# danspeech/danspeech

Hardware: AMD Instinct MI355X
Metric: audio-seconds/sec (RTFx) recognize() on 10 s clips, batch=32 (higher is better)
Workload: dtype f32 (two-term fp16 split operands, 3 MFMA products, fp32 accumulate)

## Files before the change

### danspeech_amd/_native.py

```python
import ctypes as C
import os

import numpy as np

_HERE = os.path.dirname(os.path.abspath(__file__))
LIB_PATH = os.environ.get("DSMI_LIBRARY") or os.path.join(_HERE, "lib", "libdsmi.so")

RNN_TYPES = {"gru": 0, "lstm": 1, "rnn": 2}
WINDOWS = {"hamming": 0, "hann": 1, "blackman": 2, "bartlett": 3}
PCM_DTYPES = {np.dtype(np.int16): 0, np.dtype(np.float32): 1, np.dtype(np.float64): 2}
WAV_WIDTH_DTYPE = {1: 3, 2: 0, 3: 4, 4: 5}
PCM_STEREO = 16
_PCM_BYTES = (2, 4, 8, 1, 3, 4)
PAD_MODES = {"reflect": 0, "constant": 1}
RESAMPLE_METHODS = {"polyphase": 0, "ratecv": 1}
RESAMPLE_STREAM_MAX = 256
ENDPOINT_MAX = 256
STREAM_MANY_MAX = 256
BEAM_STREAM_MANY_MAX = 4096
ALIGN_MAX_TOKENS = 4096
SPOT_MAX_TOKENS = 128
SPOT_MAX_PHRASES = 4096
SPOT_MAX_HITS = 64
SCORE_MAX_TOKENS = 2048
# ... 108 lines not shown
    "dsmi_rnn_layer": (C.c_int, [_vp, C.c_int, _vp, _vp, C.c_int, C.c_int, _vp, _vp]),
    "dsmi_head": (C.c_int, [_vp, _vp, _vp, C.c_int, C.c_int, _vp, _vp]),
    "dsmi_greedy": (C.c_int, [_vp, _vp, _vp, C.c_int, C.c_int, _vp, _vp, _vp, _vp]),
    "dsmi_greedy_enqueue": (C.c_int, [_vp, _vp, _vp, C.c_int, C.c_int, _vp]),
    "dsmi_greedy_collect": (C.c_int, [_vp, _vp, _vp, _vp]),
    "dsmi_set_profiling": (C.c_int, [_vp, C.c_int]),
    "dsmi_stage_time_us": (C.c_double, [_vp, C.c_int]),
    "dsmi_kernel_stats": (C.c_int, [_vp, C.c_int, _i64p, _i64p, C.POINTER(C.c_double), C.POINTER(C.c_double), C.POINTER(C.c_double)]),
    "dsmi_reset_kernel_stats": (C.c_int, [_vp]),
    "dsmi_debug_persist_stamps": (C.c_int, [_vp, C.c_int, C.c_int, C.c_int, _vp, C.c_int64]),
    "dsmi_debug_step_stamps": (C.c_int, [_vp, C.c_int, C.c_int, C.c_int, C.c_int, _vp, C.c_int64]),
    "dsmi_debug_last_rnn_plan": (C.c_int, [_vp, C.c_char_p, C.c_int64]),
    "dsmi_debug_xproj": (C.c_int, [_vp, _vp, C.c_int64, _vp, _vp, _vp]),
    "dsmi_debug_conv_workgroups": (C.c_int, [_vp, _vp, C.c_int32]),
    "dsmi_debug_dense_stamps": (C.c_int, [_vp, C.c_int64]),
    "dsmi_last_forward_stats": (C.c_int, [_vp, _i64p, C.POINTER(C.c_double), C.POINTER(C.c_double)]),
    "dsmi_lm_open": (C.c_int, [C.c_char_p, C.POINTER(_vp)]),
    "dsmi_lm_close": (None, [_vp]),
    "dsmi_lm_last_error": (C.c_char_p, [_vp]),
    "dsmi_lm_info": (C.c_int, [_vp, C.POINTER(C.c_int), _i64p, C.POINTER(C.c_int)]),
    "dsmi_lm_word_index": (C.c_int, [_vp, C.c_char_p]),
    "dsmi_lm_lookup": (C.c_int, [_vp, _vp, C.c_int, C.POINTER(C.c_float), C.POINTER(C.c_float)]),
    "dsmi_lm_cond_log10": (C.c_double, [_vp, _vp, C.c_int]),
    "dsmi_beam_enqueue": (C.c_int, [_vp, _vp, _vp, C.c_int, C.c_int, C.c_int, C.c_int, C.c_double, _vp]),
    "dsmi_beam_collect": (C.c_int, [_vp, _vp, _vp, _vp, _vp]),
    "dsmi_decoder_beam_stats": (C.c_int, [_vp, _vp]),
    "dsmi_debug_beam_stamps": (C.c_int, [_vp, _vp, C.c_int64]),
    "dsmi_beam_stream_create": (C.c_int, [_vp, C.c_int, C.c_int, C.c_double, C.POINTER(_vp)]),
    "dsmi_beam_stream_destroy": (None, [_vp]),
    "dsmi_beam_stream_last_error": (C.c_char_p, [_vp]),
# ... 1043 lines not shown
```

### danspeech_amd/csrc/api.hip

```cpp
#include "common.h"
#include "model.h"
#include "gate.h"

#include <algorithm>
#include <cstring>

using namespace dsmi;

static int check_lens(dsmi_model* m, const int32_t* lens, int B, int T) {
    for (int i = 0; i < B; ++i) {
        if (lens[i] < 1 || lens[i] > T) return fail(m, DSMI_ERR_INVALID, "length outside 1..T");
        if (i && lens[i] > lens[i - 1]) return fail(m, DSMI_ERR_UNSORTED, "`lengths` array must be sorted in decreasing order");
    }
    return DSMI_OK;
}

static int check_batch(dsmi_model* m, const int32_t* lens, int B, int T) {
    if (!m->finalized) return fail(m, DSMI_ERR_NOT_READY, "dsmi_model_finalize has not been called");
    if (!lens || B < 1 || T < 1) return fail(m, DSMI_ERR_INVALID, "bad batch arguments");
    return check_lens(m, lens, B, T);
}

static int run_conv(dsmi_model* m, const float* feat, int B, int T, int To, int ys, hipStream_t s, const float** out) {
    const float* x = feat;
// ... 72 lines not shown
        const char *k = std::getenv("DSMI_RNN_KERNEL"), *t = exp_env("DSMI_RING_TILES"), *c = exp_env("DSMI_DEBUG_RING_SLOTS");
        return RingEnv{k && std::string(k) == "ring4", t ? std::atoi(t) : 4, c ? std::atoi(c) : 0};
    }();
    return env;
}

static RnnPlanInput rnn_plan_input(const dsmi_model* m, int B, bool split16) {
    RnnPlanInput in;
    in.geom = m->geom; in.geom16 = m->geom16; in.have16 = m->have16; in.split16 = split16;
    in.B = B; in.n_cus = m->n_cus; in.inflight = m->inflight; in.ring_windows = m->ring_windows; in.lane = m->lane;
    in.rnn_mode = m->rnn_mode; in.persist_gen = m->persist_gen; in.rnn_kernel = m->rnn_kernel; in.ring8 = m->ring8; in.ring4 = m->ring4;
    in.ring4_small_shapes = ring_env().small_shapes; in.ring4_most = ring_env().most; in.ring_slot_cap = ring_env().slot_cap;
    return in;
}

static bool run_rnn_plan(dsmi_model* m, const RnnPlan& plan, int l, int B, int To, int dst, double sumlen, hipStream_t s) {
    const double H = m->desc.rnn_hidden_size, GH = (double)m->geom.G * m->desc.rnn_hidden_size, Dd = m->geom.D;
    if (plan.launches[0].kernel == RNN_STEPS) {
        RnnStepLaunch st = rnn_step_launch(m, l, B, To, dst);
        for (int step = 0; step < To; ++step) {
            st.step = step;
            int act = 0;
            for (int i = 0; i < B; ++i) act += step < m->host_out_lens[i] ? 1 : 0;
            st.ev = timer_arm(m, KK_STEP, (step & 7) == 3, 2.0 * Dd * GH * H * act, 4.0 * Dd * (GH * H + (double)B * (GH + 2.0 * H)));
            launch_rnn_step(st, s);
        }
        m->last_plan_x16 = false; m->last_plan_n = 1; m->last_plan[0] = plan.launches[0];
        return true;
    }
    RnnPersist16Launch p16;
    RnnPersistLaunch p8;
    if (plan.x16) p16 = persist16_launch(m, l, B, To, dst);
    else p8 = persist_launch(m, l, B, To, dst);
    const size_t cnt_words = persist_cnt_words(m, B, To, true, false);
    (void)hipMemsetAsync(m->pcnt, 0, sizeof(unsigned) * persist_cnt_words(m, B, To, plan.x16, true), s);
    static const bool ring_xcd = [] { const char* e = exp_env("DSMI_DEBUG_RING_XCD"); return !(e && e[0] == '0'); }();
    GateTurn turn;
    bool ok = true;
    for (int i = 0; i < plan.launches.size() && ok; ++i) {
        const RnnLaunch& L = plan.launches[i];
        const EvPair ev = timer_arm(m, KK_PERSIST, true, L.part * 2.0 * Dd * GH * H * sumlen, L.part * 4.0 * Dd * (GH * H + (double)To * B * (GH + 2.0 * H)));
        if (!L.join) turn.wait(m->device, s, L, m->n_cus);
        p16.ev = ev;
        switch (L.kernel) {
            case RNN_PERSIST8: p8.ev = ev; p8.d0 = L.at; p8.ny = L.n; ok = launch_rnn_persist(p8, s); break;
            case RNN_PERSIST16: p16.pgroups = L.n; p16.waves = 8; ok = launch_rnn_persist16(p16, s); break;
            case RNN_PERSIST16_HALF: p16.pgroups = L.n; p16.waves = 4; ok = launch_rnn_persist16(p16, s); break;
            case RNN_DUO: p16.pair0 = L.at; p16.npairs = L.n; ok = launch_rnn_persist_duo(p16, s); break;
            default:
                p16.tile0 = L.at; p16.ntw = L.n; p16.nwin = L.nwin;
                p16.tickets = ring_xcd ? m->pcnt + cnt_words + L.ticket : nullptr;
                ok = L.kernel == RNN_RING8 ? launch_rnn_persist_ring(p16, s) : launch_rnn_persist_ring4(p16, s);
        }
        if (!ok || i + 1 == plan.launches.size() || !plan.launches[i + 1].join) turn.record();
    }
    if (ok) {
        m->last_plan_x16 = plan.x16; m->last_plan_n = plan.launches.size();
        for (int i = 0; i < std::min(m->last_plan_n, (int)dsmi_model::kLastPlanKept); ++i) m->last_plan[i] = plan.launches[i];
    }
    return ok;
}

static void run_rnn_layer(dsmi_model* m, int l, GemmLaunch gl, int B, int To, int dst, hipStream_t s) {
    double sumlen = 0;
    for (int i = 0; i < B; ++i) sumlen += m->host_out_lens[i];
    const double GH = (double)m->geom.G * m->desc.rnn_hidden_size, Dd = m->geom.D;
    RnnPlanInput in = rnn_plan_input(m, B, m->gemm_mode == 1 && gl.w_sp);
    RnnPlan plan = plan_rnn_layer(in);
    if (plan.x16) {
        gl.w_sp = m->rnn[l].wih16_sp; gl.bias = m->rnn[l].bih16; gl.N = m->geom16.Np; gl.ldc = m->geom16.Np;
    }
    gl.ev = timer_arm(m, gl.mode == GEMM_A_CONV ? KK_GEMM0 : KK_GEMM, true, 2.0 * Dd * GH * gl.K * sumlen,
                      4.0 * ((double)gl.M * gl.K * (gl.a2 ? 2 : 1) + (double)gl.N * gl.K + (double)gl.M * gl.N));
    DenseHold hold(m->device, m->inflight, DENSE_GEMM, s);
    m->last_xp_wgs = launch_gemm(gl, s);
    m->last_xp_rows = gl.M; m->last_xp_cols = gl.ldc;
    hold.leave();
    if (run_rnn_plan(m, plan, l, B, To, dst, sumlen, s)) return;
    if (plan.x16) {
        gl.w_sp = m->rnn[l].wih_sp; gl.bias = m->rnn[l].bih; gl.N = m->geom.Np; gl.ldc = m->geom.Np; gl.ev = EvPair{};
        m->last_xp_wgs = launch_gemm(gl, s);
        m->last_xp_cols = gl.ldc;
        in.have16 = false;
        plan = plan_rnn_layer(in);
        if (run_rnn_plan(m, plan, l, B, To, dst, sumlen, s)) return;
    }
    in.rnn_mode = 0;
    (void)run_rnn_plan(m, plan_rnn_layer(in), l, B, To, dst, sumlen, s);
}

static GemmLaunch xproj_gemm(dsmi_model* m, int l, int B, int To) {
    GemmLaunch gl{};
    const RnnW& r = m->rnn[l];
// ... 303 lines not shown
```

### danspeech_amd/csrc/common.h

```cpp
#pragma once
#include <hip/hip_runtime.h>
#include <hip/hip_ext.h>
#include <atomic>
#include <cstdint>
#include <cstdio>
#include <cstdlib>
#include <string>
#include <vector>
#include <map>

#include "../../include/dsmi.h"
#include "dense_tiles.h"
#include "conv_rows.h"
#include "rnn_plan.h"

namespace dsmi {

using f32x4 = __attribute__((ext_vector_type(4))) float;
using f32x16 = __attribute__((ext_vector_type(16))) float;

constexpr int kWave = 64;
constexpr int kLdsOnceDevices = 64;

template <auto KERN>
// ... 129 lines not shown
std::vector<uint16_t> pack_whh_split(const RnnGeom& g, const float* w_hh);
bool launch_rnn_persist(const RnnPersistLaunch& p, hipStream_t s);

struct RnnPersist16Launch {
    RnnGeom g;
    const uint16_t* whh16[2];
    const float* bhh[2]; const float* xp; float* out[2];
    const int32_t* lens_dev; uint16_t* hpack16;
    unsigned* counters;
    unsigned* err;
    int B, T, pgroups;
    int waves = 8;
    int pair0 = 0, npairs = 0;
    int tile0 = 0, ntw = 0, nwin = 1;
    unsigned* tickets = nullptr;
    unsigned spin_limit = kPersistSpinLimit;
    int drop_wg = -1, drop_step = -1;
    EvPair ev;
    unsigned long long* dbg = nullptr;
};
constexpr int kPersist16Shards = 4;
constexpr int kPersist16CntWords = kPersist16Shards * 64;
std::vector<uint16_t> pack_whh16(const RnnGeom& g16, const float* w_hh);
size_t rnn_persist16_state_halfs(const RnnGeom& g16, int B);
bool launch_rnn_persist16(const RnnPersist16Launch& p, hipStream_t s);

bool launch_rnn_persist_duo(const RnnPersist16Launch& p, hipStream_t s);

bool launch_rnn_persist_ring(const RnnPersist16Launch& p, hipStream_t s);
bool launch_rnn_persist_ring4(const RnnPersist16Launch& p, hipStream_t s);
// ... 16 lines not shown
```

### danspeech_amd/csrc/gate.h

```cpp
#pragma once
#include "common.h"

#include <mutex>

struct PersistGate;

bool persist_process_lock(int device);
int persist_next_lane(int device);

class GateTurn {
public:
    void wait(int device, hipStream_t s, const dsmi::RnnLaunch& L, int n_cus);
    void record();
    void hold(int device);
private:
    PersistGate* g_ = nullptr;
    std::unique_lock<std::mutex> lk_;
    hipStream_t s_ = nullptr;
    dsmi::RnnLaunch l_;
};

enum DenseScope { DENSE_CONV_STACK, DENSE_CONV_LAYER, DENSE_GEMM };
int dense_token_limit();
class DenseHold {
public:
    DenseHold(int device, int inflight, DenseScope scope, hipStream_t s);
    void leave();
private:
    unsigned* sem_ = nullptr;
    hipStream_t s_ = nullptr;
};
```

### danspeech_amd/csrc/gate.hip

```cpp
#include "gate.h"
#include "gate_plan.h"

#include <fcntl.h>
#include <sys/file.h>
#include <unistd.h>

using namespace dsmi;

struct PersistGate { std::mutex mu; hipEvent_t ev[kMaxLanes] = {nullptr, nullptr, nullptr, nullptr}; hipEvent_t ring_ev[kRingSlots] = {nullptr, nullptr, nullptr, nullptr, nullptr};
                     hipEvent_t full_ev = nullptr;
                     unsigned* turn = nullptr;
                     DeviceGateState st;
                     int lock_fd = -1; bool lock_tried = false; int next_lane = 0; };

__global__ void turn_acquire_kernel(unsigned* turn) {
    if (threadIdx.x != 0) return;
    unsigned spins = 0;
    while (atomicCAS(turn, 0u, 1u) != 0u && ++spins < (1u << 20)) __builtin_amdgcn_s_sleep(32);
}
__global__ void turn_release_kernel(unsigned* turn) {
    if (threadIdx.x == 0) __hip_atomic_store(turn, 0u, __ATOMIC_RELEASE, __HIP_MEMORY_SCOPE_AGENT);
}

__global__ void dense_enter_kernel(unsigned* sem, unsigned limit) {
    if (threadIdx.x != 0) return;
    for (unsigned spins = 0; spins < (1u << 18); ++spins) {
// ... 4 lines not shown
    atomicAdd(sem, 1u);
}
__global__ void dense_leave_kernel(unsigned* sem) {
    if (threadIdx.x == 0) atomicSub(sem, 1u);
}
static int dense_tokens() {
    static const int k = [] {
        const char* e = std::getenv("DSMI_DENSE_TOKENS");
        if (e) return std::atoi(e);
        const char* q = std::getenv("GPU_MAX_HW_QUEUES");
        return q && std::atoi(q) >= 8 ? 1 : 0;
    }();
    return k;
}
int dense_token_limit() { return dense_tokens(); }
static int dense_scope() {
    static const int k = [] { const char* e = exp_env("DSMI_DEBUG_DENSE_SCOPE"); return e ? std::atoi(e) : 0; }();
    return k;
}

static PersistGate* persist_gate(int device) {
    static std::mutex mu;
    static std::map<int, PersistGate*> gates;
    std::lock_guard<std::mutex> lk(mu);
    auto it = gates.find(device);
    if (it != gates.end()) return it->second;
    PersistGate* g = new PersistGate();
    for (int i = 0; i < kMaxLanes; ++i)
        if (hipEventCreateWithFlags(&g->ev[i], hipEventDisableTiming) != hipSuccess) g->ev[i] = nullptr;
    for (int i = 0; i < kRingSlots; ++i)
// ... 29 lines not shown
    const char* tmp = std::getenv("TMPDIR");
    const std::string path = std::string(tmp && tmp[0] ? tmp : "/tmp") + "/dsmi-persist-" + bus + ".lock";
    const int fd = open(path.c_str(), O_CREAT | O_RDWR, 0666);
    if (fd < 0) { g->lock_fd = -2; return true; }
    if (flock(fd, LOCK_EX | LOCK_NB) != 0) { close(fd); g->lock_fd = -1; return false; }
    g->lock_fd = fd;
    return true;
}

int persist_next_lane(int device) {
    PersistGate* g = persist_gate(device);
    std::lock_guard<std::mutex> lk(g->mu);
    return g->next_lane++;
}

void GateTurn::wait(int device, hipStream_t s, const RnnLaunch& L, int n_cus) {
    if (!g_) g_ = persist_gate(device);
    lk_ = std::unique_lock<std::mutex>(g_->mu);
    s_ = s; l_ = L;
    const DeviceGateWait w = gate_plan_wait(g_->st, L, n_cus, g_->turn != nullptr);
    for (int i = 0; i < kMaxLanes; ++i)
        if ((w.lanes >> i & 1) && g_->ev[i]) (void)hipStreamWaitEvent(s, g_->ev[i], 0);
    for (int i = 0; i < kRingSlots; ++i)
        if ((w.ring >> i & 1) && g_->ring_ev[i]) (void)hipStreamWaitEvent(s, g_->ring_ev[i], 0);
    if (w.full && g_->full_ev) (void)hipStreamWaitEvent(s, g_->full_ev, 0);
    if (w.acquire) hipLaunchKernelGGL(turn_acquire_kernel, dim3(1), dim3(64), 0, s, g_->turn);
}
void GateTurn::record() {
    const DeviceGateRecord r = gate_plan_record(g_->st, l_, g_->turn != nullptr);
    if (r.release) hipLaunchKernelGGL(turn_release_kernel, dim3(1), dim3(64), 0, s_, g_->turn);
    for (int i = 0; i < kMaxLanes; ++i)
        if ((r.lanes >> i & 1) && g_->ev[i]) (void)hipEventRecord(g_->ev[i], s_);
    for (int i = 0; i < kRingSlots; ++i)
        if ((r.ring >> i & 1) && g_->ring_ev[i]) (void)hipEventRecord(g_->ring_ev[i], s_);
    if (r.full && g_->full_ev) (void)hipEventRecord(g_->full_ev, s_);
    g_->st = r.after;
    lk_.unlock();
}
void GateTurn::hold(int device) {
    if (!g_) g_ = persist_gate(device);
    lk_ = std::unique_lock<std::mutex>(g_->mu);
}

DenseHold::DenseHold(int device, int inflight, DenseScope scope, hipStream_t s) : s_(s) {
    const bool behind_token = scope == DENSE_GEMM || dense_scope() == (scope == DENSE_CONV_STACK ? 0 : 2);
    if (dense_tokens() > 0 && inflight >= 2 && behind_token) sem_ = dense_sem(device);
    if (sem_) hipLaunchKernelGGL(dense_enter_kernel, dim3(1), dim3(64), 0, s_, sem_, (unsigned)dense_tokens());
}
void DenseHold::leave() {
    if (sem_) hipLaunchKernelGGL(dense_leave_kernel, dim3(1), dim3(64), 0, s_, sem_);
}
```

### danspeech_amd/csrc/model.h

```cpp
#pragma once
#include "common.h"

struct HostTensor {
    std::vector<int64_t> shape;
    std::vector<float> data;
};

struct ConvW { float *wp = nullptr, *bias = nullptr, *bn_a = nullptr, *bn_b = nullptr; uint16_t* wp_sp = nullptr; };

struct RnnW {
    float* wih = nullptr;
    uint16_t* wih_sp = nullptr;
    float* bih = nullptr;
    float* whh[2] = {nullptr, nullptr};
    uint16_t* whh_sp[2] = {nullptr, nullptr};
    float* bhh[2] = {nullptr, nullptr};
    uint16_t* wih16_sp = nullptr; float* bih16 = nullptr; uint16_t* whh16_sp[2] = {nullptr, nullptr};
    float* bn_a = nullptr;
    float* bn_b = nullptr;
    int K = 0, ldw = 0;
};

enum KernelKind { KK_STFT = 0, KK_CONV1, KK_CONV2, KK_CONV3, KK_GEMM0, KK_GEMM, KK_STEP, KK_HEAD, KK_GREEDY, KK_BEAM, KK_PERSIST, KK_COUNT };
struct KernelTimer {
// ... 50 lines not shown
    unsigned* pcnt = nullptr;
    unsigned* perr = nullptr;
    struct FwdSlot {
        const float* feat = nullptr; float* probs = nullptr; std::vector<int32_t> lens; int B = 0, T = 0; void* stream = nullptr;
        hipEvent_t done = nullptr;
        unsigned* err_host = nullptr;
    };
    static constexpr int kFwdRing = 4;
    FwdSlot fwd[kFwdRing];
    int fwd_head = 0, fwd_count = 0;
    int recomputed = 0;
    static constexpr int kLastPlanKept = 8;
    dsmi::RnnLaunch last_plan[kLastPlanKept];
    int last_plan_n = 0;
    bool last_plan_x16 = false;
    unsigned spin_limit = dsmi::kPersistSpinLimit;
    int drop_layer = -1, drop_wg = -1, drop_step = -1;
    int lane = 0;
    static constexpr int kStage = 4;
    int32_t* lens_stage = nullptr; int stage_cap = 0, stage_next = 0;
    hipEvent_t stage_ev[kStage] = {nullptr, nullptr, nullptr, nullptr}; bool stage_used[kStage] = {false, false, false, false};
    int n_cus = 0;
    bool conv1_split = true;
    int conv_mode = 1;
    int gemm_mode = 1;
    int rnn_mode = 1;
    bool ring4 = false;
    bool ring8 = false;
    int rnn_kernel = 0;
    int persist_gen = 2;
// ... 13 lines not shown

#define HIP_OK(m, expr)                                                                   \
    do {                                                                                  \
        hipError_t e_ = (expr);                                                           \
        if (e_ != hipSuccess) {                                                           \
            (m)->err = std::string(#expr) + ": " + hipGetErrorString(e_);                 \
            return DSMI_ERR_HIP;                                                          \
        }                                                                                 \
    } while (0)

inline int fail(dsmi_model* m, int code, const std::string& msg) {
    m->err = msg;
    return code;
}

inline size_t persist_cnt_words(const dsmi_model* m, int B, int To, bool x16, bool tickets) {
    if (!x16) return (size_t)m->geom.D * dsmi::ceil_div(B, 32) * To;
    return (size_t)m->geom.D * dsmi::ceil_div(B, 16) * To * dsmi::kPersist16CntWords + (tickets ? 2 * dsmi::ceil_div(B, 16) + 2 : 0);
}

int seq_len(const dsmi_model* m, int L);
int frames_for(int To);

dsmi::EvPair timer_arm(dsmi_model* m, int kind, bool sample, double flops, double bytes);
void timer_resolve(dsmi_model* m);

void stream_batch_free(dsmi_model* m);
bool stream_persist_layer(dsmi_model* m, const dsmi::RnnPersistLaunch& pl, hipStream_t s);
dsmi::RnnPersist16Launch persist16_launch(const dsmi_model* m, int l, int B, int To, int dst);
dsmi::RnnPersistLaunch persist_launch(const dsmi_model* m, int l, int B, int To, int dst);
dsmi::RnnStepLaunch rnn_step_launch(const dsmi_model* m, int l, int B, int To, int dst);
struct RingEnv { bool small_shapes; int most, slot_cap; };
const RingEnv& ring_env();
// ... 1 lines not shown
```

### danspeech_amd/csrc/profile.hip

```cpp
#include "common.h"
#include "model.h"
#include "gate.h"

#include <algorithm>
#include <cstring>

using namespace dsmi;

EvPair timer_arm(dsmi_model* m, int kind, bool sample, double flops, double bytes) {
    EvPair ev;
    if (m->profiling < 2) return ev;
    KernelTimer& t = m->kt;
    t.launches[kind] += 1;
    t.flops[kind] += flops;
    t.bytes[kind] += bytes;
    if (!sample) return ev;
    static const int every = [] { const char* e = exp_env("DSMI_DEBUG_SAMPLE_EVERY"); const int v = e ? std::atoi(e) : 5; return v < 1 ? 1 : v; }();
    if (kind != KK_PERSIST && kind != KK_STEP && (t.launches[kind] - 1) % every != 0) return ev;
    static const int ring_every = [] { const char* e = exp_env("DSMI_DEBUG_SAMPLE_RING_EVERY"); const int v = e ? std::atoi(e) : 1; return v < 1 ? 1 : v; }();
    if (kind == KK_PERSIST && (t.launches[kind] - 1) % ring_every != 0) return ev;
    hipEvent_t e[2];
    for (int i = 0; i < 2; ++i) {
        if (!t.free_events.empty()) { e[i] = t.free_events.back(); t.free_events.pop_back(); }
        else if (hipEventCreate(&e[i]) != hipSuccess) return EvPair();
// ... 39 lines not shown
    const int64_t n = (int64_t)m->last_xp_rows * m->last_xp_cols;
    if (!xp_host || !rows || !cols || !workgroups || n == 0 || !m->xp || capacity < n) return fail(m, DSMI_ERR_INVALID, "dsmi_debug_xproj: no layer has run, or the buffer is too small");
    HIP_OK(m, hipSetDevice(m->device));
    HIP_OK(m, hipDeviceSynchronize());
    HIP_OK(m, hipMemcpy(xp_host, m->xp, sizeof(float) * (size_t)n, hipMemcpyDeviceToHost));
    *rows = m->last_xp_rows; *cols = m->last_xp_cols; *workgroups = m->last_xp_wgs;
    return DSMI_OK;
}

extern "C" int dsmi_debug_conv_workgroups(const dsmi_model* m, int32_t* workgroups, int32_t capacity) {
    if (!m || !workgroups || capacity < m->desc.conv_layers) return DSMI_ERR_INVALID;
    for (int l = 0; l < m->desc.conv_layers; ++l) workgroups[l] = m->last_conv_wgs[l];
    return m->desc.conv_layers;
}

extern "C" int dsmi_set_profiling(dsmi_model* m, int level) {
    if (!m) return DSMI_ERR_INVALID;
    m->profiling = level < 0 ? 0 : (level > 2 ? 2 : level);
    if (m->profiling == 2 && hipSetDevice(m->device) == hipSuccess)
        while (m->kt.free_events.size() < 256) {
            hipEvent_t e;
            if (hipEventCreate(&e) != hipSuccess) break;
            m->kt.free_events.push_back(e);
        }
    return DSMI_OK;
}

extern "C" int dsmi_kernel_stats(dsmi_model* m, int kind, int64_t* launches, int64_t* samples, double* avg_us,
                                 double* flops_per_launch, double* bytes_per_launch) {
    if (!m || kind < 0 || kind >= KK_COUNT) return DSMI_ERR_INVALID;
// ... 126 lines not shown
```

### danspeech_amd/csrc/rnn_persist_ring.hip

```cpp
#include "common.h"
#include "rnn_cell.h"
#include <algorithm>
#include <cstdlib>
#include <cstring>
#include <type_traits>

namespace dsmi {

namespace {

constexpr int RNT = kRingThreads;
constexpr int RU = kTileUnits;
constexpr int RB = kTileClips;
constexpr int RRP = kRingRedPitch;
constexpr int RMINT = kRingMaxTiles;

using u32x4 = __attribute__((ext_vector_type(4))) unsigned int;
using f16x8 = __attribute__((ext_vector_type(8))) _Float16;
constexpr float kLoScale = 2048.f, kLoInv = 1.f / 2048.f;

struct RingArgs {
    const uint16_t* whh[2];
    const float* bhh[2]; const float* xp; float* out[2];
    const int32_t* lens; uint16_t* hpack; unsigned* cnt; unsigned* err;
    int B, T, H, Hs, Np, nwg16, nkb;
    int ntiles, D;
    int tile0, ntw, tile_end;
    unsigned spin_limit;
    int drop_wg, drop_step;
    unsigned* tickets;
    int skip;
    unsigned long long* dbg;
};

#define RSTAMP(k)                                                                          \
    do {                                                                                   \
        if (STAMP) {                                                                       \
            __builtin_amdgcn_sched_barrier(0);                                             \
            const unsigned long long now_ = __builtin_amdgcn_s_memtime();                  \
            if ((threadIdx.x & 63) == 0) tacc[k] += now_ - clast;                          \
            clast = now_;                                                                  \
            __builtin_amdgcn_sched_barrier(0);                                             \
        }                                                                                  \
    } while (0)

// ... 28 lines not shown
    if (p.tickets && p.D == 2) {
        const int nw = (p.nwg16 + 1) >> 1;
        if (tid == 0) {
            unsigned xcc;
            asm volatile("s_getreg_b32 %0, hwreg(HW_REG_XCC_ID)" : "=s"(xcc));
            unsigned* tk = p.tickets + 2 * blockIdx.z;
            unsigned want = (xcc >> 2) & 1u;
            unsigned t = atomicAdd(&tk[want], 1u);
            if (t >= (unsigned)nw) { want ^= 1u; t = atomicAdd(&tk[want], 1u); }
            sync[30] = (int)want; sync[31] = (int)t;
        }
        __syncthreads();
        d = __builtin_amdgcn_readfirstlane(sync[30]);
        w32 = __builtin_amdgcn_readfirstlane(sync[31]);
        __syncthreads();
    }
    const int tile0 = p.tile0 + (int)blockIdx.z * p.ntw;
    const int nt = min(min(p.ntw, p.tile_end - tile0), NT);
    const int w16 = 2 * w32 + hx;
    const bool half_ok = w16 < p.nwg16;
    const int nwg32 = (p.nwg16 + 1) >> 1;
    const int GU = NG * RU;
    float* red = red_all + hx * (4 * NG * 16 * RRP);
    for (int i = tid; i < NT * RNT; i += RNT) { st_h[i] = 0.f; if (KIND == DSMI_RNN_LSTM) st_c[i] = 0.f; }
    if (tid < 32) sync[tid] = 0;
    if (STAMP && lane < 16) tacc[lane] = 0;
    if (tid < NT * 16) {
        const int tl = tid >> 4, eb = (tile0 + tl) * RB + (tid & 15);
        st_len[tid] = (tl < nt && eb < p.B) ? p.lens[eb] : 0;
    }
// ... 353 lines not shown
}

}

bool launch_rnn_persist_ring(const RnnPersist16Launch& p, hipStream_t s) {
    RingArgs a;
    for (int d = 0; d < 2; ++d) { a.whh[d] = p.whh16[d]; a.bhh[d] = p.bhh[d]; a.out[d] = p.out[d]; }
    a.xp = p.xp; a.lens = p.lens_dev; a.hpack = p.hpack16; a.cnt = p.counters; a.err = p.err;
    a.B = p.B; a.T = p.T; a.H = p.g.H; a.Hs = p.g.Kp; a.Np = p.g.Np; a.nwg16 = p.g.nwg; a.nkb = ceil_div(p.g.H, 32);
    a.ntiles = ceil_div(p.B, RB); a.D = p.g.D;
    a.tile0 = p.tile0; a.ntw = p.ntw > 0 ? p.ntw : a.ntiles - p.tile0;
    a.tile_end = std::min(a.ntiles, a.tile0 + a.ntw * std::max(p.nwin, 1));
    if (a.ntw < 1 || a.ntw > RMINT || a.tile_end <= a.tile0) return false;
    if ((size_t)p.T * p.B * p.g.Kp * 4 >= (1ull << 31)) return false;
    a.spin_limit = p.spin_limit; a.drop_wg = p.drop_wg; a.drop_step = p.drop_step; a.dbg = p.dbg; a.tickets = p.tickets;
    static const int skip = exp_env("DSMI_DEBUG_RING_SKIP") ? std::atoi(exp_env("DSMI_DEBUG_RING_SKIP")) : 0;
    a.skip = skip;
    switch (p.g.kind) {
        case DSMI_RNN_GRU: return launch_ring<DSMI_RNN_GRU>(a, s, p.ev);
        case DSMI_RNN_LSTM: return launch_ring<DSMI_RNN_LSTM>(a, s, p.ev);
        default: return launch_ring<DSMI_RNN_TANH>(a, s, p.ev);
    }
}

}
```

### danspeech_amd/csrc/rnn_persist_ring4.hip

```cpp
#include "common.h"
#include "rnn_cell.h"
#include <algorithm>
#include <cstdlib>
#include <cstring>
#include <type_traits>

namespace dsmi {

namespace {

constexpr int XNT = 256;
constexpr int XU = kTileUnits;
constexpr int XB = kTileClips;
constexpr int XMAXT = kRing4MaxTiles;

using u32x4 = __attribute__((ext_vector_type(4))) unsigned int;
using u32x2 = __attribute__((ext_vector_type(2))) unsigned int;
using f32x2 = __attribute__((ext_vector_type(2))) float;
using f16x8 = __attribute__((ext_vector_type(8))) _Float16;
constexpr float kLoScale = 2048.f, kLoInv = 1.f / 2048.f;

struct Ring4Args {
    const uint16_t* whh[2];
    const float* bhh[2]; const float* xp; float* out[2];
    const int32_t* lens; uint16_t* hpack; unsigned* cnt; unsigned* err;
    int B, T, H, Hs, Np, nwg16, nkb;
    int ntiles, D;
    int tile0, ntw, tile_end;
    unsigned spin_limit;
    int drop_wg, drop_step;
    unsigned* tickets;
    unsigned long long* dbg;
};

template <class T>
__device__ __forceinline__ const T* uni_ptr(const T* q) {
    const unsigned long long a = reinterpret_cast<unsigned long long>(q);
    const unsigned lo = __builtin_amdgcn_readfirstlane((unsigned)a), hi = __builtin_amdgcn_readfirstlane((unsigned)(a >> 32));
    return reinterpret_cast<const T*>(((unsigned long long)hi << 32) | lo);
}

__device__ __forceinline__ void ring4_barrier() { asm volatile("s_waitcnt lgkmcnt(0)\n\ts_barrier" ::: "memory"); }




// ... 23 lines not shown
        const int nw = (p.nwg16 + 1) >> 1;
        if (tid == 0) {
            unsigned xcc;
            asm volatile("s_getreg_b32 %0, hwreg(HW_REG_XCC_ID)" : "=s"(xcc));
            unsigned* tk = p.tickets + 2 * blockIdx.z;
            unsigned want = (xcc >> 2) & 1u;
            unsigned t = atomicAdd(&tk[want], 1u);
            if (t >= (unsigned)nw) { want ^= 1u; t = atomicAdd(&tk[want], 1u); }
            sync[30] = (int)want; sync[31] = (int)t;
        }
        ring4_barrier();
        d = __builtin_amdgcn_readfirstlane(sync[30]);
        w32 = __builtin_amdgcn_readfirstlane(sync[31]);
        ring4_barrier();
    }
    const int tile0 = p.tile0 + (int)blockIdx.z * p.ntw;
    const int nt = min(min(p.ntw, p.tile_end - tile0), NT);
    const int w16 = 2 * w32 + mh;
    const bool half_ok = w16 < p.nwg16;
    const int nwg32 = (p.nwg16 + 1) >> 1;
    constexpr int GU = NG * XU;
    {
        u32x4* z = reinterpret_cast<u32x4*>(xlds);
        const int n16 = (2 * sbytes + (2 * RED_BUF + 3 * 2 * NG * 256) * 4) / 16;
        for (int i = tid; i < n16; i += XNT) z[i] = u32x4{0u, 0u, 0u, 0u};
    }
    if (tid < 32) sync[tid] = 0;
    if (STAMP && lane < 8) tacc[lane] = 0;

    const int kb0 = kh ? (p.nkb + 1) / 2 : 0, kb1 = kh ? p.nkb : (p.nkb + 1) / 2;
// ... 397 lines not shown
}

}

bool launch_rnn_persist_ring4(const RnnPersist16Launch& p, hipStream_t s) {
    Ring4Args a;
    for (int d = 0; d < 2; ++d) { a.whh[d] = p.whh16[d]; a.bhh[d] = p.bhh[d]; a.out[d] = p.out[d]; }
    a.xp = p.xp; a.lens = p.lens_dev; a.hpack = p.hpack16; a.cnt = p.counters; a.err = p.err;
    a.B = p.B; a.T = p.T; a.H = p.g.H; a.Hs = p.g.Kp; a.Np = p.g.Np; a.nwg16 = p.g.nwg; a.nkb = ceil_div(p.g.H, 32);
    a.ntiles = ceil_div(p.B, XB); a.D = p.g.D;
    a.tile0 = p.tile0; a.ntw = p.ntw > 0 ? p.ntw : a.ntiles - p.tile0;
    a.tile_end = std::min(a.ntiles, a.tile0 + a.ntw * std::max(p.nwin, 1));
    if (a.ntw < 1 || a.ntw > XMAXT || a.tile_end <= a.tile0) return false;
    if ((size_t)p.T * p.B * p.g.Kp * 4 >= (1ull << 31)) return false;
    a.spin_limit = p.spin_limit; a.drop_wg = p.drop_wg; a.drop_step = p.drop_step; a.dbg = p.dbg; a.tickets = p.tickets;
    if (a.ntw > 4) {
#ifndef DSMI_EXPERIMENTS
        return false;
#else
        switch (p.g.kind) {
            case DSMI_RNN_GRU: return launch_ring4_nt<DSMI_RNN_GRU, 8>(a, s, p.ev);
            case DSMI_RNN_LSTM: return launch_ring4_nt<DSMI_RNN_LSTM, 8>(a, s, p.ev);
            default: return launch_ring4_nt<DSMI_RNN_TANH, 8>(a, s, p.ev);
        }
#endif
    }
    switch (p.g.kind) {
        case DSMI_RNN_GRU: return launch_ring4_nt<DSMI_RNN_GRU, 4>(a, s, p.ev);
        case DSMI_RNN_LSTM: return launch_ring4_nt<DSMI_RNN_LSTM, 4>(a, s, p.ev);
        default: return launch_ring4_nt<DSMI_RNN_TANH, 4>(a, s, p.ev);
// ... 5 lines not shown
```

### include/dsmi.h

```cpp
#ifndef DSMI_H
#define DSMI_H

#include <stddef.h>
#include <stdint.h>

#ifdef __cplusplus
extern "C" {
#endif
#if defined(DSMI_BUILD) && defined(__GNUC__)
#pragma GCC visibility push(default)
#endif

typedef enum {
    DSMI_OK = 0,
    DSMI_ERR_INVALID = -1,
    DSMI_ERR_CONV = -2,
    DSMI_ERR_NOT_READY = -3,
    DSMI_ERR_UNSORTED = -4,
    DSMI_ERR_HIP = -5,
    DSMI_ERR_NOMEM = -6,
    DSMI_ERR_IO = -7,
    DSMI_ERR_CAPACITY = -8,
    DSMI_ERR_TIMEOUT = -9,
    DSMI_ERR_COMM = -10,
// ... 139 lines not shown
                int32_t* ids_host, int32_t* offsets_host, int32_t* n_out_host, void* stream);
int dsmi_greedy_enqueue(dsmi_decoder* d, const float* probs_dev, const int32_t* sizes_host, int B, int T_out, void* stream);
int dsmi_greedy_collect(dsmi_decoder* d, int32_t* ids_host, int32_t* offsets_host, int32_t* n_out_host);

int dsmi_set_profiling(dsmi_model* m, int level);
int dsmi_kernel_stats(dsmi_model* m, int kind, int64_t* launches, int64_t* samples, double* avg_us,
                      double* flops_per_launch, double* bytes_per_launch);
int dsmi_reset_kernel_stats(dsmi_model* m);
int dsmi_debug_persist_stamps(dsmi_model* m, int layer, int B, int T_out, uint64_t* stamps_host, int64_t n_words);
int dsmi_debug_step_stamps(dsmi_model* m, int layer, int B, int T_out, int step, uint64_t* stamps_host,
                           int64_t n_words);
int dsmi_debug_last_rnn_plan(const dsmi_model* m, char* buf, int64_t capacity);
int dsmi_debug_xproj(dsmi_model* m, float* xp_host, int64_t capacity, int32_t* rows, int32_t* cols, int32_t* workgroups);
int dsmi_debug_conv_workgroups(const dsmi_model* m, int32_t* workgroups, int32_t capacity);
int dsmi_debug_dense_stamps(uint64_t* stamps_host, int64_t n_words);
double dsmi_stage_time_us(const dsmi_model* m, int stage);
int dsmi_last_forward_stats(const dsmi_model* m, int64_t* n_step_launches, double* step_flops,
                            double* total_flops);

int dsmi_decoder_set_lm(dsmi_decoder* d, const char* lm_path, double alpha, double beta);
int dsmi_beam(dsmi_decoder* d, const float* probs_dev, const int32_t* sizes_host, int B, int T_out,
              int beam_width, int cutoff_top_n, double cutoff_prob, int32_t* tokens_host,
              int32_t* tsteps_host, int32_t* lens_host, float* scores_host, void* stream);
int dsmi_beam_enqueue(dsmi_decoder* d, const float* probs_dev, const int32_t* sizes_host, int B, int T_out,
                      int beam_width, int cutoff_top_n, double cutoff_prob, void* stream);
int dsmi_beam_collect(dsmi_decoder* d, int32_t* tokens_host, int32_t* tsteps_host, int32_t* lens_host, float* scores_host);
int dsmi_decoder_beam_stats(const dsmi_decoder* d, int32_t* counts4);
int dsmi_debug_beam_stamps(const dsmi_decoder* d, uint64_t* stamps_host, int64_t n_words);

typedef struct dsmi_beam_stream dsmi_beam_stream;
// ... 84 lines not shown
```

Before: 61900.

## Pass dense GEMM token to ring RNN kernel and zero counters before GEMM

```diff
diff --git a/danspeech_amd/_native.py b/danspeech_amd/_native.py
--- a/danspeech_amd/_native.py
+++ b/danspeech_amd/_native.py
@@ -146,6 +146,8 @@
     "dsmi_debug_xproj": (C.c_int, [_vp, _vp, C.c_int64, _vp, _vp, _vp]),
     "dsmi_debug_conv_workgroups": (C.c_int, [_vp, _vp, C.c_int32]),
     "dsmi_debug_dense_stamps": (C.c_int, [_vp, C.c_int64]),
+    "dsmi_debug_token_pass": (C.c_int, [_vp, _vp, _vp, C.c_int32]),
+    "dsmi_debug_ring_arrival": (C.c_int, [_vp, C.c_int64]),
     "dsmi_last_forward_stats": (C.c_int, [_vp, _i64p, C.POINTER(C.c_double), C.POINTER(C.c_double)]),
     "dsmi_lm_open": (C.c_int, [C.c_char_p, C.POINTER(_vp)]),
     "dsmi_lm_close": (None, [_vp]),
diff --git a/danspeech_amd/csrc/api.hip b/danspeech_amd/csrc/api.hip
--- a/danspeech_amd/csrc/api.hip
+++ b/danspeech_amd/csrc/api.hip
@@ -110,7 +110,10 @@
     return in;
 }
 
-static bool run_rnn_plan(dsmi_model* m, const RnnPlan& plan, int l, int B, int To, int dst, double sumlen, hipStream_t s) {
+static bool rnn_ring_first(const RnnPlan& plan) { return token_pass_applies(plan.launches[0].kernel, plan.launches[0].gate, true, true); }
+
+static bool run_rnn_plan(dsmi_model* m, const RnnPlan& plan, int l, int B, int To, int dst, double sumlen, hipStream_t s,
+                         bool zeroed = false, DenseHold* pass = nullptr, unsigned long long* arrival = nullptr) {
     const double H = m->desc.rnn_hidden_size, GH = (double)m->geom.G * m->desc.rnn_hidden_size, Dd = m->geom.D;
     if (plan.launches[0].kernel == RNN_STEPS) {
         RnnStepLaunch st = rnn_step_launch(m, l, B, To, dst);
@@ -129,14 +132,18 @@
     if (plan.x16) p16 = persist16_launch(m, l, B, To, dst);
     else p8 = persist_launch(m, l, B, To, dst);
     const size_t cnt_words = persist_cnt_words(m, B, To, true, false);
-    (void)hipMemsetAsync(m->pcnt, 0, sizeof(unsigned) * persist_cnt_words(m, B, To, plan.x16, true), s);
+    if (!zeroed) (void)hipMemsetAsync(m->pcnt, 0, sizeof(unsigned) * persist_cnt_words(m, B, To, plan.x16, true), s);
     static const bool ring_xcd = [] { const char* e = exp_env("DSMI_DEBUG_RING_XCD"); return !(e && e[0] == '0'); }();
     GateTurn turn;
-    bool ok = true;
+    bool ok = true, handed = false;
+    unsigned* const pass_words = m->pcnt + cnt_words + persist_ticket_words(B);
     for (int i = 0; i < plan.launches.size() && ok; ++i) {
         const RnnLaunch& L = plan.launches[i];
         const EvPair ev = timer_arm(m, KK_PERSIST, true, L.part * 2.0 * Dd * GH * H * sumlen, L.part * 4.0 * Dd * (GH * H + (double)To * B * (GH + 2.0 * H)));
-        if (!L.join) turn.wait(m->device, s, L, m->n_cus);
+        if (!L.join) {
+            const bool kept = turn.wait(m->device, s, L, m->n_cus, i == 0 ? pass : nullptr);
+            if (i == 0 && kept) { handed = true; ++m->pass_layers[2]; if (!rnn_ring_first(plan)) ++m->pass_layers[3]; }
+        }
         p16.ev = ev;
         switch (L.kernel) {
             case RNN_PERSIST8: p8.ev = ev; p8.d0 = L.at; p8.ny = L.n; ok = launch_rnn_persist(p8, s); break;
@@ -146,9 +153,16 @@
             default:
                 p16.tile0 = L.at; p16.ntw = L.n; p16.nwin = L.nwin;
                 p16.tickets = ring_xcd ? m->pcnt + cnt_words + L.ticket : nullptr;
+                p16.token = handed && i == 0 ? pass->token() : nullptr;
+                p16.pass = p16.token ? pass_words : nullptr;
+                p16.arrival = i == 0 ? arrival : nullptr;
                 ok = L.kernel == RNN_RING8 ? launch_rnn_persist_ring(p16, s) : launch_rnn_persist_ring4(p16, s);
         }
         if (!ok || i + 1 == plan.launches.size() || !plan.launches[i + 1].join) turn.record();
+        if (handed && i == 0) {
+            if (ok) pass->leave_once(pass_words);
+            else pass->leave();
+        }
     }
     if (ok) {
         m->last_plan_x16 = plan.x16; m->last_plan_n = plan.launches.size();
@@ -168,11 +182,20 @@
     }
     gl.ev = timer_arm(m, gl.mode == GEMM_A_CONV ? KK_GEMM0 : KK_GEMM, true, 2.0 * Dd * GH * gl.K * sumlen,
                       4.0 * ((double)gl.M * gl.K * (gl.a2 ? 2 : 1) + (double)gl.N * gl.K + (double)gl.M * gl.N));
+    static const bool late_zero = [] { const char* e = exp_env("DSMI_DEBUG_LATE_ZERO"); return e && e[0] == '1'; }();
+    const bool zeroed_ahead = plan.launches[0].kernel != RNN_STEPS && !late_zero;
+    if (zeroed_ahead) (void)hipMemsetAsync(m->pcnt, 0, sizeof(unsigned) * persist_cnt_words(m, B, To, plan.x16, true), s);
     DenseHold hold(m->device, m->inflight, DENSE_GEMM, s);
     m->last_xp_wgs = launch_gemm(gl, s);
     m->last_xp_rows = gl.M; m->last_xp_cols = gl.ldc;
-    hold.leave();
-    if (run_rnn_plan(m, plan, l, B, To, dst, sumlen, s)) return;
+    static_assert(RNN_RING8 == 5 && RNN_RING4 == 6 && GATE_RING == 2, "token_pass_applies names them by number");
+    const bool held = hold.token() != nullptr;
+    const bool pass = token_pass_applies(plan.launches[0].kernel, plan.launches[0].gate, held, token_to_ring());
+    if (held) { ++m->pass_layers[0]; if (rnn_ring_first(plan)) ++m->pass_layers[1]; }
+    unsigned long long* const arrival = held && rnn_ring_first(plan) ? ring_arrival_slot() : nullptr;
+    if (!pass) hold.leave(arrival);
+    else hold.mark(arrival);
+    if (run_rnn_plan(m, plan, l, B, To, dst, sumlen, s, zeroed_ahead, pass ? &hold : nullptr, arrival)) return;
     if (plan.x16) {
         gl.w_sp = m->rnn[l].wih_sp; gl.bias = m->rnn[l].bih; gl.N = m->geom.Np; gl.ldc = m->geom.Np; gl.ev = EvPair{};
         m->last_xp_wgs = launch_gemm(gl, s);
diff --git a/danspeech_amd/csrc/common.h b/danspeech_amd/csrc/common.h
--- a/danspeech_amd/csrc/common.h
+++ b/danspeech_amd/csrc/common.h
@@ -167,6 +167,8 @@
     int pair0 = 0, npairs = 0;
     int tile0 = 0, ntw = 0, nwin = 1;
     unsigned* tickets = nullptr;
+    unsigned* token = nullptr; unsigned* pass = nullptr;
+    unsigned long long* arrival = nullptr;
     unsigned spin_limit = kPersistSpinLimit;
     int drop_wg = -1, drop_step = -1;
     EvPair ev;
diff --git a/danspeech_amd/csrc/gate.h b/danspeech_amd/csrc/gate.h
--- a/danspeech_amd/csrc/gate.h
+++ b/danspeech_amd/csrc/gate.h
@@ -4,13 +4,14 @@
 #include <mutex>
 
 struct PersistGate;
+class DenseHold;
 
 bool persist_process_lock(int device);
 int persist_next_lane(int device);
 
 class GateTurn {
 public:
-    void wait(int device, hipStream_t s, const dsmi::RnnLaunch& L, int n_cus);
+    bool wait(int device, hipStream_t s, const dsmi::RnnLaunch& L, int n_cus, DenseHold* pass = nullptr);
     void record();
     void hold(int device);
 private:
@@ -22,10 +23,19 @@
 
 enum DenseScope { DENSE_CONV_STACK, DENSE_CONV_LAYER, DENSE_GEMM };
 int dense_token_limit();
+bool token_to_ring();
+bool dense_token_read(int device, unsigned* value);
+constexpr int kRingArrivalWords = 4, kRingArrivalSlots = 8192;
+unsigned long long* ring_arrival_slot();
+int ring_arrival_read(unsigned long long* host, long long n_words);
 class DenseHold {
 public:
     DenseHold(int device, int inflight, DenseScope scope, hipStream_t s);
     void leave();
+    void leave(unsigned long long* stamps);
+    void mark(unsigned long long* stamps);
+    unsigned* token() const { return sem_; }
+    void leave_once(unsigned* pass);
 private:
     unsigned* sem_ = nullptr;
     hipStream_t s_ = nullptr;
diff --git a/danspeech_amd/csrc/gate.hip b/danspeech_amd/csrc/gate.hip
--- a/danspeech_amd/csrc/gate.hip
+++ b/danspeech_amd/csrc/gate.hip
@@ -1,5 +1,6 @@
 #include "gate.h"
 #include "gate_plan.h"
+#include "token_pass.h"
 
 #include <fcntl.h>
 #include <sys/file.h>
@@ -7,9 +8,11 @@
 
 using namespace dsmi;
 
+struct GateOwner { hipStream_t stream = nullptr; bool recorded = false; };
 struct PersistGate { std::mutex mu; hipEvent_t ev[kMaxLanes] = {nullptr, nullptr, nullptr, nullptr}; hipEvent_t ring_ev[kRingSlots] = {nullptr, nullptr, nullptr, nullptr, nullptr};
                      hipEvent_t full_ev = nullptr;
                      unsigned* turn = nullptr;
+                     GateOwner ev_by[kMaxLanes], ring_by[kRingSlots], full_by;
                      DeviceGateState st;
                      int lock_fd = -1; bool lock_tried = false; int next_lane = 0; };
 
@@ -44,6 +47,16 @@
     return k;
 }
 int dense_token_limit() { return dense_tokens(); }
+constexpr bool kTokenToRingDefault = false;
+__global__ void dense_leave_once_kernel(unsigned* sem, unsigned* pass) {
+    if (threadIdx.x != 0) return;
+    const unsigned old = __hip_atomic_fetch_or(pass + kTokenPassFlag, (unsigned)TOKEN_PASS_BACKSTOP, __ATOMIC_ACQ_REL, __HIP_MEMORY_SCOPE_AGENT);
+    if (token_pass_claim(old, TOKEN_PASS_BACKSTOP).give_back) atomicSub(sem, 1u);
+}
+bool token_to_ring() {
+    static const bool k = [] { const char* e = std::getenv("DSMI_TOKEN_TO_RING"); return e && e[0] ? std::atoi(e) != 0 : kTokenToRingDefault; }();
+    return k;
+}
 static int dense_scope() {
     static const int k = [] { const char* e = exp_env("DSMI_DEBUG_DENSE_SCOPE"); return e ? std::atoi(e) : 0; }();
     return k;
@@ -103,26 +116,34 @@
     return g->next_lane++;
 }
 
-void GateTurn::wait(int device, hipStream_t s, const RnnLaunch& L, int n_cus) {
+bool GateTurn::wait(int device, hipStream_t s, const RnnLaunch& L, int n_cus, DenseHold* pass) {
     if (!g_) g_ = persist_gate(device);
     lk_ = std::unique_lock<std::mutex>(g_->mu);
     s_ = s; l_ = L;
     const DeviceGateWait w = gate_plan_wait(g_->st, L, n_cus, g_->turn != nullptr);
+    if (pass && pass->token()) {
+        auto pending_elsewhere = [&](hipEvent_t e, const GateOwner& by) { return e && by.recorded && by.stream != s && hipEventQuery(e) != hipSuccess; };
+        bool foreign = w.acquire || (w.full && pending_elsewhere(g_->full_ev, g_->full_by));
+        for (int i = 0; i < kMaxLanes; ++i) foreign |= (w.lanes >> i & 1) && pending_elsewhere(g_->ev[i], g_->ev_by[i]);
+        for (int i = 0; i < kRingSlots; ++i) foreign |= (w.ring >> i & 1) && pending_elsewhere(g_->ring_ev[i], g_->ring_by[i]);
+        if (foreign) { pass->leave(); pass = nullptr; }
+    } else pass = nullptr;
     for (int i = 0; i < kMaxLanes; ++i)
         if ((w.lanes >> i & 1) && g_->ev[i]) (void)hipStreamWaitEvent(s, g_->ev[i], 0);
     for (int i = 0; i < kRingSlots; ++i)
         if ((w.ring >> i & 1) && g_->ring_ev[i]) (void)hipStreamWaitEvent(s, g_->ring_ev[i], 0);
     if (w.full && g_->full_ev) (void)hipStreamWaitEvent(s, g_->full_ev, 0);
     if (w.acquire) hipLaunchKernelGGL(turn_acquire_kernel, dim3(1), dim3(64), 0, s, g_->turn);
+    return pass != nullptr;
 }
 void GateTurn::record() {
     const DeviceGateRecord r = gate_plan_record(g_->st, l_, g_->turn != nullptr);
     if (r.release) hipLaunchKernelGGL(turn_release_kernel, dim3(1), dim3(64), 0, s_, g_->turn);
     for (int i = 0; i < kMaxLanes; ++i)
-        if ((r.lanes >> i & 1) && g_->ev[i]) (void)hipEventRecord(g_->ev[i], s_);
+        if ((r.lanes >> i & 1) && g_->ev[i]) { (void)hipEventRecord(g_->ev[i], s_); g_->ev_by[i] = GateOwner{s_, true}; }
     for (int i = 0; i < kRingSlots; ++i)
-        if ((r.ring >> i & 1) && g_->ring_ev[i]) (void)hipEventRecord(g_->ring_ev[i], s_);
-    if (r.full && g_->full_ev) (void)hipEventRecord(g_->full_ev, s_);
+        if ((r.ring >> i & 1) && g_->ring_ev[i]) { (void)hipEventRecord(g_->ring_ev[i], s_); g_->ring_by[i] = GateOwner{s_, true}; }
+    if (r.full && g_->full_ev) { (void)hipEventRecord(g_->full_ev, s_); g_->full_by = GateOwner{s_, true}; }
     g_->st = r.after;
     lk_.unlock();
 }
@@ -139,3 +160,55 @@
 void DenseHold::leave() {
     if (sem_) hipLaunchKernelGGL(dense_leave_kernel, dim3(1), dim3(64), 0, s_, sem_);
 }
+#ifdef DSMI_EXPERIMENTS
+__global__ void dense_stamp_kernel(unsigned* sem, unsigned long long* stamps) {
+    if (threadIdx.x != 0) return;
+    const unsigned long long now = __builtin_amdgcn_s_memrealtime();
+    stamps[3] = now;
+    if (sem) { stamps[2] = now; atomicSub(sem, 1u); }
+}
+static std::mutex g_arrival_mu;
+static unsigned long long* g_arrival = nullptr;
+static int g_arrival_next = 0;
+unsigned long long* ring_arrival_slot() {
+    static const bool on = [] { const char* e = exp_env("DSMI_DEBUG_RING_ARRIVAL"); return e && std::atoi(e) != 0; }();
+    if (!on) return nullptr;
+    std::lock_guard<std::mutex> lk(g_arrival_mu);
+    if (!g_arrival) {
+        std::vector<unsigned long long> init((size_t)kRingArrivalWords * kRingArrivalSlots, 0ull);
+        for (int i = 0; i < kRingArrivalSlots; ++i) init[(size_t)i * kRingArrivalWords] = ~0ull;
+        if (hipMalloc((void**)&g_arrival, init.size() * sizeof(unsigned long long)) != hipSuccess) { g_arrival = nullptr; return nullptr; }
+        (void)hipMemcpy(g_arrival, init.data(), init.size() * sizeof(unsigned long long), hipMemcpyHostToDevice);
+    }
+    if (g_arrival_next >= kRingArrivalSlots) return nullptr;
+    return g_arrival + (size_t)kRingArrivalWords * g_arrival_next++;
+}
+int ring_arrival_read(unsigned long long* host, long long n_words) {
+    std::lock_guard<std::mutex> lk(g_arrival_mu);
+    const int n = (int)std::min<long long>(g_arrival_next, n_words / kRingArrivalWords);
+    if (n <= 0) return 0;
+    if (hipDeviceSynchronize() != hipSuccess ||
+        hipMemcpy(host, g_arrival, sizeof(unsigned long long) * kRingArrivalWords * (size_t)n, hipMemcpyDeviceToHost) != hipSuccess) return DSMI_ERR_HIP;
+    return n;
+}
+void DenseHold::leave(unsigned long long* stamps) {
+    if (!stamps) return leave();
+    if (sem_) hipLaunchKernelGGL(dense_stamp_kernel, dim3(1), dim3(64), 0, s_, sem_, stamps);
+}
+void DenseHold::mark(unsigned long long* stamps) {
+    if (stamps) hipLaunchKernelGGL(dense_stamp_kernel, dim3(1), dim3(64), 0, s_, (unsigned*)nullptr, stamps);
+}
+#else
+unsigned long long* ring_arrival_slot() { return nullptr; }
+int ring_arrival_read(unsigned long long*, long long) { return 0; }
+void DenseHold::leave(unsigned long long*) { leave(); }
+void DenseHold::mark(unsigned long long*) {}
+#endif
+void DenseHold::leave_once(unsigned* pass) {
+    if (sem_) hipLaunchKernelGGL(dense_leave_once_kernel, dim3(1), dim3(64), 0, s_, sem_, pass);
+}
+bool dense_token_read(int device, unsigned* value) {
+    unsigned* sem = dense_sem(device);
+    if (!sem || hipSetDevice(device) != hipSuccess || hipDeviceSynchronize() != hipSuccess) return false;
+    return hipMemcpy(value, sem, sizeof(unsigned), hipMemcpyDeviceToHost) == hipSuccess;
+}
diff --git a/danspeech_amd/csrc/model.h b/danspeech_amd/csrc/model.h
--- a/danspeech_amd/csrc/model.h
+++ b/danspeech_amd/csrc/model.h
@@ -1,5 +1,6 @@
 #pragma once
 #include "common.h"
+#include "token_pass.h"
 
 struct HostTensor {
     std::vector<int64_t> shape;
@@ -88,6 +89,7 @@
     dsmi::RnnLaunch last_plan[kLastPlanKept];
     int last_plan_n = 0;
     bool last_plan_x16 = false;
+    int64_t pass_layers[4] = {0, 0, 0, 0};
     unsigned spin_limit = dsmi::kPersistSpinLimit;
     int drop_layer = -1, drop_wg = -1, drop_step = -1;
     int lane = 0;
@@ -131,9 +133,11 @@
     return code;
 }
 
+inline size_t persist_ticket_words(int B) { return 2 * (size_t)dsmi::ceil_div(B, 16) + 2; }
 inline size_t persist_cnt_words(const dsmi_model* m, int B, int To, bool x16, bool tickets) {
     if (!x16) return (size_t)m->geom.D * dsmi::ceil_div(B, 32) * To;
-    return (size_t)m->geom.D * dsmi::ceil_div(B, 16) * To * dsmi::kPersist16CntWords + (tickets ? 2 * dsmi::ceil_div(B, 16) + 2 : 0);
+    return (size_t)m->geom.D * dsmi::ceil_div(B, 16) * To * dsmi::kPersist16CntWords +
+           (tickets ? (size_t)dsmi::round_up((int)(persist_ticket_words(B) + dsmi::kTokenPassWords), 4) : 0);
 }
 
 int seq_len(const dsmi_model* m, int L);
diff --git a/danspeech_amd/csrc/profile.hip b/danspeech_amd/csrc/profile.hip
--- a/danspeech_amd/csrc/profile.hip
+++ b/danspeech_amd/csrc/profile.hip
@@ -77,6 +77,19 @@
     return m->desc.conv_layers;
 }
 
+extern "C" int dsmi_debug_token_pass(dsmi_model* m, int64_t* token, int64_t* layers, int32_t capacity) {
+    if (!m || !token || !layers || capacity < 4) return DSMI_ERR_INVALID;
+    for (int i = 0; i < 4; ++i) layers[i] = m->pass_layers[i];
+    unsigned word = 0;
+    *token = dense_token_read(m->device, &word) ? (int64_t)word : -1;
+    return token_to_ring() ? 1 : 0;
+}
+
+extern "C" int dsmi_debug_ring_arrival(uint64_t* stamps_host, int64_t n_words) {
+    if (!stamps_host || n_words < 0) return DSMI_ERR_INVALID;
+    return ring_arrival_read(reinterpret_cast<unsigned long long*>(stamps_host), n_words);
+}
+
 extern "C" int dsmi_set_profiling(dsmi_model* m, int level) {
     if (!m) return DSMI_ERR_INVALID;
     m->profiling = level < 0 ? 0 : (level > 2 ? 2 : level);
diff --git a/danspeech_amd/csrc/rnn_persist_ring.hip b/danspeech_amd/csrc/rnn_persist_ring.hip
--- a/danspeech_amd/csrc/rnn_persist_ring.hip
+++ b/danspeech_amd/csrc/rnn_persist_ring.hip
@@ -1,5 +1,6 @@
 #include "common.h"
 #include "rnn_cell.h"
+#include "token_pass.h"
 #include <algorithm>
 #include <cstdlib>
 #include <cstring>
@@ -29,6 +30,10 @@
     unsigned spin_limit;
     int drop_wg, drop_step;
     unsigned* tickets;
+    unsigned* token; unsigned* pass;
+#ifdef DSMI_EXPERIMENTS
+    unsigned long long* arrival;
+#endif
     int skip;
     unsigned long long* dbg;
 };
@@ -87,6 +92,27 @@
         d = __builtin_amdgcn_readfirstlane(sync[30]);
         w32 = __builtin_amdgcn_readfirstlane(sync[31]);
         __syncthreads();
+    }
+#ifdef DSMI_EXPERIMENTS
+    unsigned long long arrived_at = 0;
+    if (p.arrival && tid == 0) {
+        arrived_at = __builtin_amdgcn_s_memrealtime();
+        atomicMin(p.arrival, arrived_at);
+        atomicMax(p.arrival + 1, arrived_at);
+    }
+#endif
+    if (p.token && tid == 0) {
+        const unsigned grid = gridDim.x * gridDim.y * gridDim.z;
+        const unsigned before = __hip_atomic_fetch_add(p.pass + kTokenPassArrived, 1u, __ATOMIC_RELAXED, __HIP_MEMORY_SCOPE_AGENT);
+        if (token_pass_last(before, grid)) {
+            const unsigned old = __hip_atomic_fetch_or(p.pass + kTokenPassFlag, (unsigned)TOKEN_PASS_LAST_ARRIVAL, __ATOMIC_RELAXED, __HIP_MEMORY_SCOPE_AGENT);
+            if (token_pass_claim(old, TOKEN_PASS_LAST_ARRIVAL).give_back) {
+                __hip_atomic_fetch_sub(p.token, 1u, __ATOMIC_RELAXED, __HIP_MEMORY_SCOPE_AGENT);
+#ifdef DSMI_EXPERIMENTS
+                if (p.arrival) p.arrival[2] = arrived_at;
+#endif
+            }
+        }
     }
     const int tile0 = p.tile0 + (int)blockIdx.z * p.ntw;
     const int nt = min(min(p.ntw, p.tile_end - tile0), NT);
@@ -470,6 +496,10 @@
     if (a.ntw < 1 || a.ntw > RMINT || a.tile_end <= a.tile0) return false;
     if ((size_t)p.T * p.B * p.g.Kp * 4 >= (1ull << 31)) return false;
     a.spin_limit = p.spin_limit; a.drop_wg = p.drop_wg; a.drop_step = p.drop_step; a.dbg = p.dbg; a.tickets = p.tickets;
+    a.token = p.pass ? p.token : nullptr; a.pass = p.pass;
+#ifdef DSMI_EXPERIMENTS
+    a.arrival = p.arrival;
+#endif
     static const int skip = exp_env("DSMI_DEBUG_RING_SKIP") ? std::atoi(exp_env("DSMI_DEBUG_RING_SKIP")) : 0;
     a.skip = skip;
     switch (p.g.kind) {
diff --git a/danspeech_amd/csrc/rnn_persist_ring4.hip b/danspeech_amd/csrc/rnn_persist_ring4.hip
--- a/danspeech_amd/csrc/rnn_persist_ring4.hip
+++ b/danspeech_amd/csrc/rnn_persist_ring4.hip
@@ -1,5 +1,6 @@
 #include "common.h"
 #include "rnn_cell.h"
+#include "token_pass.h"
 #include <algorithm>
 #include <cstdlib>
 #include <cstring>
@@ -30,6 +31,10 @@
     unsigned spin_limit;
     int drop_wg, drop_step;
     unsigned* tickets;
+    unsigned* token; unsigned* pass;
+#ifdef DSMI_EXPERIMENTS
+    unsigned long long* arrival;
+#endif
     unsigned long long* dbg;
 };
 
@@ -83,6 +88,27 @@
         w32 = __builtin_amdgcn_readfirstlane(sync[31]);
         ring4_barrier();
     }
+#ifdef DSMI_EXPERIMENTS
+    unsigned long long arrived_at = 0;
+    if (p.arrival && tid == 0) {
+        arrived_at = __builtin_amdgcn_s_memrealtime();
+        atomicMin(p.arrival, arrived_at);
+        atomicMax(p.arrival + 1, arrived_at);
+    }
+#endif
+    if (p.token && tid == 0) {
+        const unsigned grid = gridDim.x * gridDim.y * gridDim.z;
+        const unsigned before = __hip_atomic_fetch_add(p.pass + kTokenPassArrived, 1u, __ATOMIC_RELAXED, __HIP_MEMORY_SCOPE_AGENT);
+        if (token_pass_last(before, grid)) {
+            const unsigned old = __hip_atomic_fetch_or(p.pass + kTokenPassFlag, (unsigned)TOKEN_PASS_LAST_ARRIVAL, __ATOMIC_RELAXED, __HIP_MEMORY_SCOPE_AGENT);
+            if (token_pass_claim(old, TOKEN_PASS_LAST_ARRIVAL).give_back) {
+                __hip_atomic_fetch_sub(p.token, 1u, __ATOMIC_RELAXED, __HIP_MEMORY_SCOPE_AGENT);
+#ifdef DSMI_EXPERIMENTS
+                if (p.arrival) p.arrival[2] = arrived_at;
+#endif
+            }
+        }
+    }
     const int tile0 = p.tile0 + (int)blockIdx.z * p.ntw;
     const int nt = min(min(p.ntw, p.tile_end - tile0), NT);
     const int w16 = 2 * w32 + mh;
@@ -510,6 +536,10 @@
     if (a.ntw < 1 || a.ntw > XMAXT || a.tile_end <= a.tile0) return false;
     if ((size_t)p.T * p.B * p.g.Kp * 4 >= (1ull << 31)) return false;
     a.spin_limit = p.spin_limit; a.drop_wg = p.drop_wg; a.drop_step = p.drop_step; a.dbg = p.dbg; a.tickets = p.tickets;
+    a.token = p.pass ? p.token : nullptr; a.pass = p.pass;
+#ifdef DSMI_EXPERIMENTS
+    a.arrival = p.arrival;
+#endif
     if (a.ntw > 4) {
 #ifndef DSMI_EXPERIMENTS
         return false;
diff --git a/danspeech_amd/csrc/token_pass.h b/danspeech_amd/csrc/token_pass.h
--- /dev/null
+++ b/danspeech_amd/csrc/token_pass.h
@@ -0,0 +1,27 @@
+#pragma once
+
+#if defined(__HIPCC__) || defined(__CUDACC__)
+#define DSMI_TOKEN_PASS_FN __host__ __device__ inline
+#else
+#define DSMI_TOKEN_PASS_FN inline
+#endif
+
+namespace dsmi {
+
+constexpr int kTokenPassArrived = 0, kTokenPassFlag = 1, kTokenPassWords = 2;
+enum TokenPassWho : unsigned { TOKEN_PASS_LAST_ARRIVAL = 1u, TOKEN_PASS_BACKSTOP = 2u };
+
+struct TokenPassClaim {
+    bool give_back;
+    unsigned flag;
+};
+DSMI_TOKEN_PASS_FN TokenPassClaim token_pass_claim(unsigned old_flag, unsigned who) {
+    return TokenPassClaim{old_flag == 0u, old_flag | who};
+}
+DSMI_TOKEN_PASS_FN bool token_pass_last(unsigned before, unsigned grid) { return before + 1u == grid; }
+
+DSMI_TOKEN_PASS_FN bool token_pass_applies(int first_kernel, int first_gate, bool token_held, bool switch_on) {
+    return switch_on && token_held && first_gate == 2 && (first_kernel == 5 || first_kernel == 6);
+}
+
+}
diff --git a/include/dsmi.h b/include/dsmi.h
--- a/include/dsmi.h
+++ b/include/dsmi.h
@@ -177,6 +177,8 @@
 int dsmi_debug_xproj(dsmi_model* m, float* xp_host, int64_t capacity, int32_t* rows, int32_t* cols, int32_t* workgroups);
 int dsmi_debug_conv_workgroups(const dsmi_model* m, int32_t* workgroups, int32_t capacity);
 int dsmi_debug_dense_stamps(uint64_t* stamps_host, int64_t n_words);
+int dsmi_debug_token_pass(dsmi_model* m, int64_t* token, int64_t* layers, int32_t capacity);
+int dsmi_debug_ring_arrival(uint64_t* stamps_host, int64_t n_words);
 double dsmi_stage_time_us(const dsmi_model* m, int stage);
 int dsmi_last_forward_stats(const dsmi_model* m, int64_t* n_step_launches, double* step_flops,
                             double* total_flops);
```

After: 62190 (median of 3 runs). Within noise of the previous version (+0.5%).
